# jackra1n/raytracer-rust

Hardware: NVIDIA B200
Metric: Mpaths/s (semesterbild 800x600x256spp, depth 30) (higher is better)
Workload: dtype f32

## Files before the change

### raytracer-rust_b200/csrc/pt_bvh8.h

```cpp
#pragma once
#include "pt_math.h"
#include "pt_types.h"

namespace pt {

struct MeshHit {
  float t;
  uint32_t tri;
  uint32_t order;
};

PT_HD float box_rcp(float x) {
#if defined(__CUDA_ARCH__)
  float r;
  asm("rcp.approx.ftz.f32 %0, %1;" : "=f"(r) : "f"(x));
  return r;
#else
  return 1.0f / x;
#endif
}

template <int J>
PT_HD float byte_as_unit_float(uint32_t packed) {
#if defined(__CUDA_ARCH__)
// ... 22 lines not shown
  uint32_t octinv;
  uint2 ng;
  uint2 tg;
  uint2 tg2;
};

PT_HD void trav_begin(TravState &s, V3 o, V3 d, float t_min, float t_max) {
  s.o = o;
  s.d = d;
  s.idx = box_rcp(d.x), s.idy = box_rcp(d.y), s.idz = box_rcp(d.z);
  s.t_min = t_min;
  s.best_t = t_max;
  s.best_order = 0u;
  s.best_tri = 0xffffffffu;
  const uint32_t sx = f2u(d.x) >> 31, sy = f2u(d.y) >> 31, sz = f2u(d.z) >> 31;
  s.octinv = 7u - (sx | (sy << 1) | (sz << 2));
  s.ng = make_uint2(0u, 0x80000000u);
  s.tg = make_uint2(0u, 0u);
  s.tg2 = make_uint2(0u, 0u);
}
PT_HD bool trav_has_node(const TravState &s) { return s.ng.y > 0x00FFFFFFu; }
PT_HD bool trav_has_tri(const TravState &s) { return s.tg.y != 0u; }

template <bool COUNT>
PT_HD void trav_node(const DMesh &m, TravState &s, uint2 *stack, int &sp, TraversalCounters *ctr) {
  const uint32_t hits = s.ng.y, imask = hits & 0xffu;
  const int bit = 31 - clz32(hits);
  s.ng.y &= ~(1u << bit);
  if (s.ng.y > 0x00FFFFFFu) stack[sp++] = s.ng;
  const uint32_t slot = (uint32_t)(bit - 24) ^ s.octinv;
  const uint32_t rel = (uint32_t)popc32(imask & ~(0xFFFFFFFFu << slot));
  const float4 *np = m.nodes + (size_t)(s.ng.x + rel) * 5;
  const float4 q0 = ldg4(np), q1 = ldg4(np + 1), q2 = ldg4(np + 2), q3 = ldg4(np + 3), q4 = ldg4(np + 4);
  if (COUNT) ctr->nodes++;

  const uint32_t e = f2u(q0.w);
  const float adjx = u2f(((e & 0xffu) + 15u) << 23) * s.idx;
  const float adjy = u2f((((e >> 8) & 0xffu) + 15u) << 23) * s.idy;
  const float adjz = u2f((((e >> 16) & 0xffu) + 15u) << 23) * s.idz;
  const float orgx = (q0.x - s.o.x) * s.idx - adjx, orgy = (q0.y - s.o.y) * s.idy - adjy, orgz = (q0.z - s.o.z) * s.idz - adjz;

  const bool sx = (f2u(s.d.x) >> 31) != 0u, sy = (f2u(s.d.y) >> 31) != 0u, sz = (f2u(s.d.z) >> 31) != 0u;
  const uint32_t lox0 = f2u(q2.x), lox1 = f2u(q2.y), loy0 = f2u(q2.z), loy1 = f2u(q2.w);
  const uint32_t loz0 = f2u(q3.x), loz1 = f2u(q3.y), hix0 = f2u(q3.z), hix1 = f2u(q3.w);
  const uint32_t hiy0 = f2u(q4.x), hiy1 = f2u(q4.y), hiz0 = f2u(q4.z), hiz1 = f2u(q4.w);
  const uint32_t nx[2] = {sx ? hix0 : lox0, sx ? hix1 : lox1}, fx[2] = {sx ? lox0 : hix0, sx ? lox1 : hix1};
  const uint32_t ny[2] = {sy ? hiy0 : loy0, sy ? hiy1 : loy1}, fy[2] = {sy ? loy0 : hiy0, sy ? loy1 : hiy1};
  const uint32_t nz[2] = {sz ? hiz0 : loz0, sz ? hiz1 : loz1}, fz[2] = {sz ? loz0 : hiz0, sz ? loz1 : hiz1};
  const uint32_t meta[2] = {f2u(q1.z), f2u(q1.w)};
  const uint32_t octinv4 = s.octinv * 0x01010101u;

  uint32_t hitmask = 0u;
#pragma unroll
  for (int h = 0; h < 2; h++) {
    const uint32_t meta4 = meta[h];
    const uint32_t is_inner4 = (meta4 & (meta4 << 1)) & 0x10101010u;
    const uint32_t inner_mask4 = (is_inner4 >> 4) * 0xffu;
    const uint32_t bit_index4 = (meta4 ^ (octinv4 & inner_mask4)) & 0x1f1f1f1fu;
    const uint32_t child_bits4 = (meta4 >> 5) & 0x07070707u;
#define PT_CHILD2(J)                                                                                                  \
  {                                                                                                                   \
    float tnx0, tnx1, tny0, tny1, tnz0, tnz1, tfx0, tfx1, tfy0, tfy1, tfz0, tfz1;                                     \
    fma2_bcast(tnx0, tnx1, byte_as_unit_float<J>(nx[h]), byte_as_unit_float<J + 1>(nx[h]), adjx, orgx);               \
    fma2_bcast(tny0, tny1, byte_as_unit_float<J>(ny[h]), byte_as_unit_float<J + 1>(ny[h]), adjy, orgy);               \
    fma2_bcast(tnz0, tnz1, byte_as_unit_float<J>(nz[h]), byte_as_unit_float<J + 1>(nz[h]), adjz, orgz);               \
    fma2_bcast(tfx0, tfx1, byte_as_unit_float<J>(fx[h]), byte_as_unit_float<J + 1>(fx[h]), adjx, orgx);               \
    fma2_bcast(tfy0, tfy1, byte_as_unit_float<J>(fy[h]), byte_as_unit_float<J + 1>(fy[h]), adjy, orgy);               \
    fma2_bcast(tfz0, tfz1, byte_as_unit_float<J>(fz[h]), byte_as_unit_float<J + 1>(fz[h]), adjz, orgz);               \
             \
    const float tn0 = fmaxf(fmaxf(tnx0, tny0), fmaxf(tnz0, s.t_min)), tf0 = fminf(fminf(tfx0, tfy0), fminf(tfz0, s.best_t)); \
    const float tn1 = fmaxf(fmaxf(tnx1, tny1), fmaxf(tnz1, s.t_min)), tf1 = fminf(fminf(tfx1, tfy1), fminf(tfz1, s.best_t)); \
    if (tn0 <= tf0) hitmask |= ((child_bits4 >> (8 * (J))) & 0xffu) << ((bit_index4 >> (8 * (J))) & 0xffu);           \
    if (tn1 <= tf1) hitmask |= ((child_bits4 >> (8 * (J + 1))) & 0xffu) << ((bit_index4 >> (8 * (J + 1))) & 0xffu);   \
  }
    PT_CHILD2(0) PT_CHILD2(2)
#undef PT_CHILD
  }
  s.ng.x = f2u(q1.x);
  s.ng.y = (hitmask & 0xFF000000u) | (e >> 24);
  const uint2 leaf_hits = make_uint2(f2u(q1.y), hitmask & 0x00FFFFFFu);
  if (s.tg.y == 0u) s.tg = leaf_hits;
  else s.tg2 = leaf_hits;
}

template <bool COUNT>
PT_HD void trav_tri(const DMesh &m, TravState &s, TraversalCounters *ctr) {
  const int bit = 31 - clz32(s.tg.y);
  const float4 *tp = m.tris + (size_t)(s.tg.x + (uint32_t)bit) * 3;
  s.tg.y &= ~(1u << bit);
  if (s.tg.y == 0u) {
    s.tg = s.tg2;
    s.tg2 = make_uint2(0u, 0u);
  }
  const float4 t0 = ldg4(tp), t1 = ldg4(tp + 1), t2 = ldg4(tp + 2);
  if (COUNT) ctr->tris++;
  const V3 v0 = v3(t0.x, t0.y, t0.z), edge1 = v3(t1.x, t1.y, t1.z), edge2 = v3(t2.x, t2.y, t2.z);
  const V3 h = cross(s.d, edge2);
  const float a = dot(edge1, h);
  if (fabsf(a) < kEps) return;
  const float f = 1.0f / a;
  const V3 sv = s.o - v0;
  const float u = f * dot(sv, h);
  if (!(0.0f <= u && u <= 1.0f)) return;
  const V3 q = cross(sv, edge1);
  const float v = f * dot(s.d, q);
  if (v < 0.0f || u + v > 1.0f) return;
  const float t = f * dot(edge2, q);
  if (!(t > s.t_min)) return;
  const uint32_t order = f2u(t1.w);
  if (t < s.best_t || (t == s.best_t && order < s.best_order)) {
    s.best_t = t;
    s.best_order = order;
    s.best_tri = f2u(t0.w);
  }
}

template <bool COUNT>
PT_HD bool bvh8_closest(const DMesh &m, V3 o, V3 d, float t_min, float t_max, MeshHit &out, TraversalCounters *ctr) {
  TravState s;
  trav_begin(s, o, d, t_min, t_max);
  uint2 stack[kTraversalStack];
  int sp = 0;
  for (;;) {
    if (trav_has_tri(s)) {
      trav_tri<COUNT>(m, s, ctr);
    } else if (trav_has_node(s)) {
      trav_node<COUNT>(m, s, stack, sp, ctr);
    } else {
      if (sp == 0) break;
      s.ng = stack[--sp];
    }
  }
  if (s.best_tri == 0xffffffffu) return false;
  out.t = s.best_t;
  out.tri = s.best_tri;
  out.order = s.best_order;
  return true;
}

}
```

### raytracer-rust_b200/csrc/pt_prims.h

```cpp
#pragma once
#include "pt_bvh8.h"
#include "pt_math.h"
#include "pt_types.h"

namespace pt {

PT_HD void set_face_normal(Hit &h, V3 ray_d, V3 outward) {
  bool front = dot(ray_d, outward) < 0.0f;
  V3 n = front ? outward : -outward;
  h.front_face = front ? 1 : 0;
  h.nx = n.x;
  h.ny = n.y;
  h.nz = n.z;
}
PT_HD void set_pos(Hit &h, V3 p) {
  h.px = p.x;
  h.py = p.y;
  h.pz = p.z;
}

PT_HD bool hit_sphere(const float *f, const Ray &ray, float t_min, float t_max, Hit &h) {
  const float4 cr = ld4(reinterpret_cast<const float4 *>(f));
  const V3 center = v3(cr.x, cr.y, cr.z);
  const float radius = cr.w;
// ... 102 lines not shown
    }
  }
  const M4 w2o = load_m4(f);
  const V3 nw = normalized(mat_t_vector(w2o, n));
  set_face_normal(h, ray.d, nw);
}
PT_HD bool hit_cube(const float *f, const Ray &ray, float t_min, float t_max, Hit &h) {
  if (!hit_cube_t(f, ray, t_min, t_max, h)) return false;
  cube_finish_normal(f, ray, h);
  return true;
}

struct MeshRay {
  V3 o, d_raw, d;
};
template <bool PACKED = true>
PT_HD MeshRay mesh_object_ray(const float *w2o_f, const Ray &ray) {
  const M4 w2o = load_m4(w2o_f);
  MeshRay r;
  mat_point_vector<PACKED>(w2o, ray.o, ray.d, r.o, r.d_raw);
  r.d = normalized(normalized(r.d_raw));
  return r;
}
PT_HD bool mesh_root_may_hit(const DMesh &mesh, const MeshRay &r, float t_min, float t_max) {
  const float idx = box_rcp(r.d.x), idy = box_rcp(r.d.y), idz = box_rcp(r.d.z);
  const float ax = (mesh.root_lo[0] - r.o.x) * idx, bx = (mesh.root_hi[0] - r.o.x) * idx;
  const float ay = (mesh.root_lo[1] - r.o.y) * idy, by = (mesh.root_hi[1] - r.o.y) * idy;
  const float az = (mesh.root_lo[2] - r.o.z) * idz, bz = (mesh.root_hi[2] - r.o.z) * idz;
  const float tn = fmaxf(fmaxf(fminf(ax, bx), fminf(ay, by)), fmaxf(fminf(az, bz), t_min));
  const float tf = fminf(fminf(fmaxf(ax, bx), fmaxf(ay, by)), fminf(fmaxf(az, bz), t_max));
  return tn <= tf;
}

PT_HD bool mesh_finish(const float *f, float4 nq, const Ray &ray, const MeshRay &mr, const MeshHit &mh, float t_min, float t_max,
                       Hit &h) {
  const M4 w2o = load_m4(f), o2w = load_m4(f + 16);
  const V3 o = mr.o, d = mr.d;
  const V3 p_obj = o + d * mh.t;
  V3 n_obj = v3(nq.x, nq.y, nq.z);
  if (!(dot(d, n_obj) < 0.0f)) n_obj = -n_obj;
  const V3 pw = mat_point(o2w, p_obj);
  const V3 nw = normalized(mat_t_vector(w2o, n_obj));
  const float t_world = mh.t * length(mr.d_raw) / length(ray.d);
  if (t_world < t_min || t_world > t_max) return false;
  h.t = t_world;
  h.triangle = (int32_t)mh.tri;
  set_pos(h, pw);
  set_face_normal(h, ray.d, nw);
  return true;
}

PT_HD bool mesh_finish(const float *f, const DMesh &mesh, const Ray &ray, const MeshRay &mr, const MeshHit &mh, float t_min,
                       float t_max, Hit &h) {
  return mesh_finish(f, ldg4(mesh.normals + mh.order), ray, mr, mh, t_min, t_max, h);
// ... 44 lines not shown
```

### raytracer-rust_b200/csrc/pt_wavefront.cuh

```cuda
#pragma once
#include <cuda_runtime.h>

#include "../../include/ptcore.h"
#include "pt_adaptive.h"
#include "pt_bsdf.h"
#include "pt_philox.h"
#include "pt_prims.h"

namespace ptw {
using namespace pt;

constexpr int kBlock = 256;
constexpr int kSegPerSM = 4;
constexpr uint32_t kRefillLanes = 8;
constexpr uint32_t kNoSteal = 0x80000000u;
constexpr unsigned long long kNoTriHit = ~0ull;

struct Ctl {
  unsigned long long next_path;
  unsigned long long total_paths;
  unsigned long long rays;
  unsigned long long nodes, tris, mesh_rays;
  uint32_t n_active;
  uint32_t sync_timeouts;
  uint32_t iterations[2];
};

struct SegRange {
  uint32_t seg0;
  uint32_t n_seg;
  uint32_t half;
  uint32_t trav_seq, trav_parts;
  uint32_t *flags;
  uint32_t stage_id;
  uint32_t flag_wait;
  uint32_t *trav_counter;
};

struct RenderParams {
  DCamera cam;
  int32_t width, height;
  int32_t max_depth;
  int32_t sample_begin, n_samples;
  int32_t tiles_x, n_my_tiles, tile_mod, tile_rem;
  uint32_t row_mult;
  uint64_t seed;
  const uint32_t *pixel_list;
  uint32_t n_list;
};

struct Buffers {
  float4 *ray_o;
  float4 *ray_d;
  float4 *beta;
// ... 70 lines not shown
    const int type = ob->type;
    bool hit;
    if (type == OBJ_MESH) {
      const MeshRay mr = mesh_object_ray(ob->f, ray);
      if (!mesh_root_may_hit(sc.meshes[ob->mesh], mr, t_min, closest)) continue;
      park_ray = mr;
      return k;
    }
    if (type == OBJ_SPHERE) hit = hit_sphere(ob->f, ray, t_min, closest, best);
    else if (type == OBJ_QUAD) hit = hit_quad(ob->f, ray, t_min, closest, best);
    else if (type == OBJ_CUBE) hit = hit_cube_t(ob->f, ray, t_min, closest, best);
    else hit = hit_plane(ob->f, ray, t_min, closest, best);
    if (hit) {
      improved = true;
      closest = best.t;
      best.object = k;
      best.triangle = -1;
      best.material = ob->hit_bits;
    }
  }
  return -1;
}

__device__ __forceinline__ void finish_hit(const DObject *objs, const Ray &ray, Hit &best) {
  if (best.front_face == kCubeNormalPending) cube_finish_normal(objs[best.object].f, ray, best);
}

constexpr int kSmemObjects = 24;
template <bool kSharedObjs>
__device__ __forceinline__ const DObject *stage_objects(const DScene &sc, DObject *s_objs) {
  if (!kSharedObjs) return sc.objects;
  const uint4 *src = reinterpret_cast<const uint4 *>(sc.objects);
  uint4 *dst = reinterpret_cast<uint4 *>(s_objs);
  const int n16 = sc.n_objects * (int)(sizeof(DObject) / 16);
  for (int i = threadIdx.x; i < n16; i += blockDim.x) dst[i] = src[i];
  return s_objs;
}

__device__ __forceinline__ void park_tasks(uint32_t *s_ntask, const TaskQ &tq, int par, uint32_t seg_base, int park, uint32_t i,
                                           const MeshRay &mr, float closest) {
  const uint32_t lane = threadIdx.x & 31u;
  const uint32_t mask = __ballot_sync(0xffffffffu, park >= 0);
  if (mask == 0u) return;
  uint32_t slot0 = 0;
  if (lane == 0) slot0 = atomicAdd(s_ntask, (uint32_t)__popc(mask));
  slot0 = __shfl_sync(0xffffffffu, slot0, 0);
  if (park >= 0) {
    const uint32_t slot = seg_base + slot0 + (uint32_t)__popc(mask & ((1u << lane) - 1u));
    tq.ray[par][slot] = make_uint2(i, (uint32_t)park);
    tq.o[par][slot] = make_float4(mr.o.x, mr.o.y, mr.o.z, closest);
    tq.d[par][slot] = make_float4(mr.d.x, mr.d.y, mr.d.z, 0.0f);
    tq.res[par][slot] = kNoTriHit;
  }
}

template <bool kSharedObjs>
__device__ __forceinline__ void stage_pre(uint32_t seg, uint32_t n_seg, const DScene &sc, const ExtendOut &out, const TaskQ &tq,
                                          float t_min, float t_max) {
  __shared__ uint32_t s_ntask;
  __shared__ __align__(16) DObject s_objs[kSmemObjects];
  const uint32_t tid = threadIdx.x;
  const uint32_t n = out.b.cnt[seg], seg_base = seg * out.b.cap;
  if (tid == 0) s_ntask = 0;
  const DObject *objs = kSharedObjs ? s_objs : sc.objects;
  stage_objects<kSharedObjs>(sc, s_objs);
  __syncthreads();
  for (uint32_t c0 = 0; c0 < n; c0 += (uint32_t)kBlock) {
    const uint32_t i = seg_base + c0 + tid;
    int park = -1;
    MeshRay mr;
    float closest = t_max;
    if (c0 + tid < n) {
      const float4 o4 = out.b.ray_o[i], d4 = out.b.ray_d[i];
      const Ray ray{v3(o4.x, o4.y, o4.z), v3(d4.x, d4.y, d4.z)};
      Hit best;
      bool improved = false;
      park = scan_objects(sc, objs, ray, t_min, closest, best, improved, 0, mr);
      if (improved) finish_hit(objs, ray, best);
      if (improved) write_hit(out, i, best);
      else write_miss(out, i);
    }
    park_tasks(&s_ntask, tq, 0, seg_base, park, i, mr, closest);
  }
  __syncthreads();
  if (tid == 0 && tq.cnt) tq.cnt[seg] = s_ntask;
  (void)n_seg;
}

template <bool COUNT>
__device__ __forceinline__ void stage_traverse(uint32_t seg, uint32_t n_seg, Ctl *ctl, const DScene &sc, const TaskQ &tq, int round,
                                               float t_min, uint32_t cap, uint32_t refill_arg, uint32_t part = 0u, uint32_t parts = 1u) {
  __shared__ uint32_t s_cur;
  const uint32_t n_all = tq.cnt[(uint32_t)round * n_seg + seg];
  const uint32_t first = (uint32_t)((unsigned long long)n_all * part / parts);
  const uint32_t n = (uint32_t)((unsigned long long)n_all * (part + 1u) / parts) - first, seg_base = seg * cap + first;
  const int par = round & 1;
  const uint32_t lane = threadIdx.x & 31u;
  const uint32_t lt_mask = (1u << lane) - 1u;
  const uint32_t refill_lanes = refill_arg & ~kNoSteal;
  const bool steal = (refill_arg & kNoSteal) == 0u;
  const uint32_t quota = (n >= (uint32_t)kBlock || !steal) ? 32u : max(1u, (n + (uint32_t)(kBlock / 32) - 1u) / (uint32_t)(kBlock / 32));
  if (threadIdx.x == 0) s_cur = 0;
  __syncthreads();
  TraversalCounters tc{0u, 0u, 0u};
  TravState s;
  DMesh mesh;
  mesh.nodes = nullptr, mesh.tris = nullptr;
  uint2 stack[kTraversalStack];
  int sp = 0, sb = 0;
  bool active = false;
  uint32_t task = 0;
  bool exhausted = n == 0u;
  s.ng = make_uint2(0u, 0u);
  for (;;) {
    const uint32_t idle = __ballot_sync(0xffffffffu, !active);
    if (!exhausted && (idle == 0xffffffffu || (uint32_t)__popc(idle) >= refill_lanes)) {
      const uint32_t cnt = min((uint32_t)__popc(idle), quota);
      uint32_t base = 0;
      if (lane == 0) base = atomicAdd(&s_cur, cnt);
      base = __shfl_sync(0xffffffffu, base, 0);
      const uint32_t my_rank = (uint32_t)__popc(idle & lt_mask);
      if (!active && my_rank < cnt) {
        const uint32_t j = base + my_rank;
        if (j < n) {
          const uint32_t slot = seg_base + j;
          const uint2 rk = tq.ray[par][slot];
          const float4 o4 = tq.o[par][slot], d4 = __ldcs(&tq.d[par][slot]);
          const DMesh *gm = sc.meshes + sc.objects[rk.y].mesh;
          mesh.nodes = gm->nodes;
          mesh.tris = gm->tris;
          trav_begin(s, v3(o4.x, o4.y, o4.z), v3(d4.x, d4.y, d4.z), t_min, o4.w);
          sp = sb = 0;
          task = slot;
          active = true;
          if (COUNT) tc.mesh_rays++;
        }
      }
      if (base + cnt >= n) exhausted = true;
    } else if (steal && exhausted && idle != 0u && idle != 0xffffffffu) {
      const bool can_give = active && (sp > sb || __popc(s.ng.y >> 24) >= 2);
      const uint32_t donors = __ballot_sync(0xffffffffu, can_give);
      if (donors != 0u) {
        const uint32_t pairs = (uint32_t)min(__popc(idle), __popc(donors));
        const bool give = can_give && (uint32_t)__popc(donors & lt_mask) < pairs;
        const uint32_t my_idle_rank = (uint32_t)__popc(idle & lt_mask);
        const bool take = !active && my_idle_rank < pairs;
        uint2 entry = make_uint2(0u, 0u);
        if (give) {
          if (sp > sb) {
            entry = stack[sb++];
          } else {
            const uint32_t pend = s.ng.y & 0xFF000000u, bit = pend & (0u - pend);
            entry = make_uint2(s.ng.x, bit | (s.ng.y & 0xffu));
            s.ng.y &= ~bit;
          }
        }
        const int src = take ? (int)__fns(donors, 0u, (int)my_idle_rank + 1) : (int)lane;
        const float ox = __shfl_sync(0xffffffffu, s.o.x, src), oy = __shfl_sync(0xffffffffu, s.o.y, src), oz = __shfl_sync(0xffffffffu, s.o.z, src);
// ... 15 lines not shown
          mesh.nodes = reinterpret_cast<const float4 *>(pn);
          mesh.tris = reinterpret_cast<const float4 *>(ptri);
          task = tk;
          sp = sb = 0;
          active = true;
        }
      }
    }
    if (__ballot_sync(0xffffffffu, active) == 0u) {
      if (exhausted) break;
      continue;
    }
    if (active) {
      if (!trav_has_node(s)) {
        if (sp > sb) {
          s.ng = stack[--sp];
        } else if (!trav_has_tri(s)) {
          if (s.best_tri != 0xffffffffu) atomicMin(&tq.res[par][task], ((unsigned long long)f2u(s.best_t) << 32) | (unsigned long long)s.best_order);
          active = false;
          s.ng.y = 0u;
        }
        if (sp == sb) sp = sb = 0;
      }
      if (active && trav_has_node(s) && s.tg2.y == 0u) trav_node<COUNT>(mesh, s, stack, sp, &tc);
      if (active && trav_has_tri(s)) trav_tri<COUNT>(mesh, s, &tc);
    }
  }
  if (COUNT) {
    atomicAdd(&ctl->nodes, (unsigned long long)tc.nodes);
    atomicAdd(&ctl->tris, (unsigned long long)tc.tris);
    atomicAdd(&ctl->mesh_rays, (unsigned long long)tc.mesh_rays);
  }
}

template <bool kSharedObjs>
__device__ __forceinline__ void stage_post(uint32_t seg, uint32_t n_seg, const DScene &sc, const ExtendOut &out, const TaskQ &tq,
                                           int round, float t_min, float t_max) {
  __shared__ uint32_t s_ntask;
  __shared__ __align__(16) DObject s_objs[kSmemObjects];
  const uint32_t tid = threadIdx.x;
  const uint32_t n = tq.cnt[(uint32_t)round * n_seg + seg], seg_base = seg * out.b.cap;
  const int par = round & 1;
  if (tid == 0) s_ntask = 0;
  const DObject *objs = kSharedObjs ? s_objs : sc.objects;
  stage_objects<kSharedObjs>(sc, s_objs);
  __syncthreads();
  for (uint32_t c0 = 0; c0 < n; c0 += (uint32_t)kBlock) {
    const uint32_t j = seg_base + c0 + tid;
    int park = -1;
    MeshRay mr;
    float closest = t_max;
    uint32_t i = 0;
    if (c0 + tid < n) {
      const uint2 rk = tq.ray[par][j];
      const unsigned long long res = tq.res[par][j];
      i = rk.x;
      const int k = (int)rk.y;
      const DObject *ob = objs + k;
      const bool tri_hit = res != kNoTriHit;
      const uint32_t order = (uint32_t)res;
      const float4 o4 = out.b.ray_o[i], d4 = out.b.ray_d[i];
      closest = tq.o[par][j].w;
      float4 nq = make_float4(0.0f, 0.0f, 0.0f, 0.0f);
      if (tri_hit) nq = ldg4(sc.meshes[ob->mesh].normals + order);
      const Ray ray{v3(o4.x, o4.y, o4.z), v3(d4.x, d4.y, d4.z)};
      Hit best;
      best.triangle = -1;
      bool improved = false;
      if (tri_hit) {
        const MeshRay omr = mesh_object_ray<false>(ob->f, ray);
        MeshHit mh;
        mh.t = u2f((uint32_t)(res >> 32)), mh.tri = f2u(nq.w), mh.order = order;
        Hit tmp;
        if (mesh_finish(ob->f, nq, ray, omr, mh, t_min, closest, tmp)) {
          improved = true;
          closest = tmp.t;
          best = tmp;
          best.object = k;
          best.material = ob->hit_bits;
        }
      }
      park = scan_objects(sc, objs, ray, t_min, closest, best, improved, k + 1, mr);
      if (improved) finish_hit(objs, ray, best);
      if (improved) write_hit(out, i, best);
    }
    park_tasks(&s_ntask, tq, par ^ 1, seg_base, park, i, mr, closest);
  }
  __syncthreads();
  if (tid == 0) tq.cnt[(uint32_t)(round + 1) * n_seg + seg] = s_ntask;
}

constexpr int kShadeClasses = 11;
constexpr int kShadeWindow = 2048;
constexpr int kShadeGroups = kShadeWindow / kBlock;

__device__ __forceinline__ uint32_t block_rank(bool flag, uint32_t *s_warp , uint32_t *total) {
  const uint32_t lane = threadIdx.x & 31u, warp = threadIdx.x >> 5;
  const uint32_t mask = __ballot_sync(0xffffffffu, flag);
  if (lane == 0) s_warp[warp] = (uint32_t)__popc(mask);
  __syncthreads();
  if (threadIdx.x == 0) {
    uint32_t tot = 0;
    for (int w = 0; w < kBlock / 32; w++) {
      const uint32_t c = s_warp[w];
      s_warp[w] = tot;
      tot += c;
    }
    s_warp[kBlock / 32] = tot;
  }
  __syncthreads();
  *total = s_warp[kBlock / 32];
  return s_warp[warp] + (uint32_t)__popc(mask & ((1u << lane) - 1u));
// ... 307 lines not shown
  else segment_wait(sr, seg, ctl);
}
__device__ __forceinline__ void stage_end(const SegRange &sr, uint32_t seg) {
  if (sr.flags == nullptr) return;
  __syncthreads();
  if (threadIdx.x == 0) st_release_u32(sr.flags + seg, sr.stage_id);
}

__global__ void __launch_bounds__(kBlock, kSegPerSM) k_extend_pre(Ctl *ctl, SegRange sr, DScene sc, ExtendOut out, TaskQ tq, float t_min,
                                                                  float t_max, volatile uint32_t *progress, uint32_t seq) {
  const uint32_t seg = sr.seg0 + blockIdx.x;
  stage_begin(sr, seg, ctl);
  if (threadIdx.x == 0) {
    const uint32_t n = out.b.cnt[seg];
    if (n) {
      atomicAdd(&ctl->rays, (unsigned long long)n);
      atomicMax(&ctl->iterations[0], seq);
    }
    if (progress && blockIdx.x == 0) {
      *progress = seq << 2 | (ctl->next_path >= ctl->total_paths ? 2u : 0u) | (ctl->n_active == 0u ? 1u : 0u);
      __threadfence_system();
    }
  }
  if (sc.n_objects <= kSmemObjects) stage_pre<true>(seg, sr.n_seg, sc, out, tq, t_min, t_max);
  else stage_pre<false>(seg, sr.n_seg, sc, out, tq, t_min, t_max);
  stage_end(sr, seg);
}
template <bool COUNT>
__global__ void __launch_bounds__(kBlock, kSegPerSM) k_traverse(Ctl *ctl, SegRange sr, DScene sc, TaskQ tq, int round, float t_min,
                                                                uint32_t cap, uint32_t refill_lanes) {
  if (sr.trav_parts <= 1u) {
    stage_begin(sr, sr.seg0 + blockIdx.x, ctl);
    stage_traverse<COUNT>(sr.seg0 + blockIdx.x, sr.n_seg, ctl, sc, tq, round, t_min, cap, refill_lanes);
    stage_end(sr, sr.seg0 + blockIdx.x);
    return;
  }
  asm volatile("griddepcontrol.launch_dependents;" ::: "memory");
  if (sr.flags == nullptr || sr.flag_wait == 0u) asm volatile("griddepcontrol.wait;" ::: "memory");
  __shared__ uint32_t s_item;
  if (threadIdx.x == 0) s_item = blockIdx.x;
  __syncthreads();
  for (;;) {
    {
      const uint32_t item = s_item;
      if (item >= sr.n_seg * sr.trav_parts) break;
      const uint32_t seg = sr.seg0 + item % sr.n_seg;
      segment_wait(sr, seg, ctl);
      stage_traverse<COUNT>(seg, sr.n_seg, ctl, sc, tq, round, t_min, cap, refill_lanes, item / sr.n_seg, sr.trav_parts);
    }
    __syncthreads();
    if (threadIdx.x == 0) {
      if (sr.flags) {
        const uint32_t seg = sr.seg0 + s_item % sr.n_seg;
        __threadfence();
        if (atomicInc(sr.flags + 2u * sr.n_seg + seg, sr.trav_parts - 1u) == sr.trav_parts - 1u) {
          __threadfence();
          st_release_u32(sr.flags + seg, sr.stage_id);
        }
      }
      s_item = gridDim.x + atomicAdd(sr.trav_counter, 1u);
    }
    __syncthreads();
  }
}
__global__ void __launch_bounds__(kBlock, kSegPerSM) k_extend_post(Ctl *ctl, SegRange sr, DScene sc, ExtendOut out, TaskQ tq, int round,
                                                                   float t_min, float t_max) {
  stage_begin(sr, sr.seg0 + blockIdx.x, ctl);
  if (sc.n_objects <= kSmemObjects) stage_post<true>(sr.seg0 + blockIdx.x, sr.n_seg, sc, out, tq, round, t_min, t_max);
  else stage_post<false>(sr.seg0 + blockIdx.x, sr.n_seg, sc, out, tq, round, t_min, t_max);
  stage_end(sr, sr.seg0 + blockIdx.x);
}
template <int Mode, bool List = false>
__global__ void __launch_bounds__(kBlock, kSegPerSM) k_shade(Ctl *ctl, SegRange sr, DScene sc, RenderParams rp, Buffers b, Film film) {
  stage_begin(sr, sr.seg0 + blockIdx.x, ctl);
  stage_shade<Mode, List>(sr.seg0 + blockIdx.x, sr.n_seg, sr.flags ? sr.flags + sr.n_seg : nullptr, ctl, sc, rp, b, film);
  stage_end(sr, sr.seg0 + blockIdx.x);
}

__global__ void k_film_to_accum(Film film, size_t n_pixels, float *accum) {
  const size_t i = (size_t)blockIdx.x * blockDim.x + threadIdx.x;
  if (i >= n_pixels * 3) return;
  const size_t px = i / 3;
  accum[i] += film_value(film.sum[i], film.flags[px], (int)(i - px * 3));
}
__global__ void k_resolve(const float *rgb, size_t n_pixels, float scale, uint32_t *out) {
  const size_t i = (size_t)blockIdx.x * blockDim.x + threadIdx.x;
  if (i < n_pixels) out[i] = resolve_pixel(rgb[i * 3] * scale, rgb[i * 3 + 1] * scale, rgb[i * 3 + 2] * scale);
}
__global__ void k_resolve_film(Film film, size_t n_pixels, float scale, const int32_t *counts, float *rgb, uint32_t *packed) {
  const size_t p = (size_t)blockIdx.x * blockDim.x + threadIdx.x;
  if (p >= n_pixels) return;
  if (counts) scale = 1.0f / (float)counts[p];
// ... 122 lines not shown
```

### raytracer-rust_b200/csrc/ptcore.cu

```cuda
#include <cuda_runtime.h>
#include <dlfcn.h>
#include <nccl.h>

#include <algorithm>
#include <chrono>
#include <memory>
#include <mutex>
#include <thread>
#include <cstdio>
#include <cstdlib>
#include <cstring>
#include <deque>
#include <functional>
#include <string>
#include <vector>

#include <cub/device/device_select.cuh>

#include "../../include/ptcore.h"
#include "pt_build_dev.h"
#include "pt_scene_host.h"
#include "pt_wavefront.cuh"

using namespace pt;
// ... 167 lines not shown
constexpr int kTravParts = 4;

enum Stage { ST_PRE = 0, ST_TRAVERSE, ST_POST, ST_SHADE, ST_COUNT };

template <typename... KArgs, typename... Args>
void launch_stage(bool pdl, cudaStream_t stream, uint32_t segments, void (*kernel)(KArgs...), Args &&...args) {
  cudaLaunchAttribute attr;
  attr.id = cudaLaunchAttributeProgrammaticStreamSerialization;
  attr.val.programmaticStreamSerializationAllowed = 1;
  cudaLaunchConfig_t cfg;
  memset(&cfg, 0, sizeof(cfg));
  cfg.gridDim = dim3(segments), cfg.blockDim = dim3(kBlock), cfg.dynamicSmemBytes = 0, cfg.stream = stream;
  cfg.attrs = pdl ? &attr : nullptr, cfg.numAttrs = pdl ? 1 : 0;
  CK(cudaLaunchKernelEx(&cfg, kernel, std::forward<Args>(args)...));
}

uint32_t traverse_refill_arg() {
  const char *r = getenv("PTC_REFILL"), *st = getenv("PTC_STEAL");
  return (r ? (uint32_t)atoi(r) : kRefillLanes) | ((st && atoi(st) == 0) ? kNoSteal : 0u);
}

int launch_extend(cudaStream_t stream, uint32_t segments, int rounds, Ctl *ctl, const DScene &ds, const ExtendOut &eo, const TaskQ &tq,
                  float t_min, float t_max, bool counters) {
  const SegRange sr{0u, segments, 0u, 0u, 1u};
  k_extend_pre<<<segments, kBlock, 0, stream>>>(ctl, sr, ds, eo, tq, t_min, t_max, nullptr, 0u);
  for (int r = 0; r < rounds; r++) {
    const SegRange tsr{0u, segments, 0u, (uint32_t)r, 1u};
    if (counters) k_traverse<true><<<segments, kBlock, 0, stream>>>(ctl, tsr, ds, tq, r, t_min, eo.b.cap, traverse_refill_arg());
    else k_traverse<false><<<segments, kBlock, 0, stream>>>(ctl, tsr, ds, tq, r, t_min, eo.b.cap, traverse_refill_arg());
    k_extend_post<<<segments, kBlock, 0, stream>>>(ctl, sr, ds, eo, tq, r, t_min, t_max);
  }
  return 1 + 2 * rounds;
}

void require_committed(const ptc_scene *s) {
  if (!s) throw std::invalid_argument("null scene");
  if (!s->committed) throw std::logic_error("scene not committed (call ptc_scene_commit first)");
}

void check_render_args(const ptc_camera *cam, const ptc_render_settings *st, bool has_output) {
  if (!cam || !st || !has_output) throw std::invalid_argument("null argument");
  if (st->width <= 0 || st->height <= 0 || st->spp <= 0) throw std::invalid_argument("bad render settings");
  if ((int64_t)st->width * st->height > (int64_t)0x3fffffff) throw std::invalid_argument("image too large");
  if ((st->flags & PTC_FLAG_NEE_SKY) && !(st->flags & PTC_FLAG_NEE)) throw std::invalid_argument("PTC_FLAG_NEE_SKY needs PTC_FLAG_NEE");
}

void sample_range(const ptc_render_settings *st, int &begin, int &end) {
// ... 128 lines not shown
    if (tev_used == s->timing_events.size()) {
      cudaEvent_t e;
      CK(cudaEventCreate(&e));
      s->timing_events.push_back(e);
    }
    return s->timing_events[tev_used++];
  };
  std::vector<int> mark_stage;
  const auto mark = [&](int stage) {
    CK(cudaEventRecord(tev(), stream));
    mark_stage.push_back(stage);
  };

  CK(cudaEventRecord(ev_begin, stream));
  uint64_t launches = 0;
  const uint32_t refill = traverse_refill_arg();
  auto is_done = [](const Ctl &c) { return c.n_active == 0 && c.sync_timeouts == 0 && c.next_path >= c.total_paths; };
  static const bool pdl_on = getenv("PTC_PDL") ? atoi(getenv("PTC_PDL")) != 0 : true;
  const bool pdl = pdl_on && !timing;
  if (init.total_paths != 0) {
    const bool dataflow = getenv("PTC_DATAFLOW") ? atoi(getenv("PTC_DATAFLOW")) != 0 : true;
    uint32_t stage_id = 0;
    auto seg_range = [&](uint32_t trav_seq_, uint32_t trav_parts_) {
      SegRange r{0u, segments, 0u, trav_seq_, trav_parts_, s->ws.seg_flags.p, ++stage_id, (dataflow && stage_id > 1u) ? 1u : 0u, nullptr};
      if (trav_parts_ > 1u) r.trav_counter = s->ws.trav_counters.p + trav_seq_;
      return r;
    };
    int64_t mesh_tris = 0;
    for (const auto &mb : s->hs.meshes) mesh_tris += mb->n;
    const char *tp_env = getenv("PTC_TRAV_PARTS");
    const uint32_t trav_parts_bulk = tp_env ? (uint32_t)std::max(1, atoi(tp_env)) : (mesh_tris >= kHeavyMeshTriangles ? (uint32_t)kTravParts : 1u);
    if (trav_parts_bulk > 1u) CK(cudaMemsetAsync(s->ws.trav_counters.p, 0, kTravCounters * sizeof(uint32_t), stream));
    uint32_t trav_seq = 0;
    bool draining = false;
    int flip = 0;
    const bool progress_on = getenv("PTC_PROGRESS") ? atoi(getenv("PTC_PROGRESS")) != 0 : true;
    uint32_t *d_progress = nullptr;
    if (progress_on) {
      CK(cudaHostGetDevicePointer((void **)&d_progress, s->h_progress, 0));
      *(volatile uint32_t *)s->h_progress = 0u;
    }
    uint64_t it = 0;
    auto run_extend = [&]() {
      const ExtendOut eo{bufs[flip], nullptr};
      if (timing) mark(ST_PRE);
      launch_stage(pdl, stream, segments, k_extend_pre, s->d_ctl.p, seg_range(0u, 1u), s->ds, eo, tq, kEps, INFINITY,
                   (volatile uint32_t *)d_progress, (uint32_t)(it + 1));
// ... 910 lines not shown
```

Measured before the change: 3168.

## Test mesh BVH root node during object scan before parking traversal tasks

The extend pre/post stages now run the full 8-wide root-node child test inline, from a shared-memory copy of each mesh's root node, before parking a ray as a traversal task. Rays that hit no root child skip the mesh entirely and continue scanning further objects. Parked tasks carry the precomputed root hit mask, so the traversal kernel enters the root directly instead of reloading and retesting it. This removes task-queue writes and traversal work for rays that miss every child, at the cost of extra ALU work and shared-memory staging in the extend stages, plus a looped object scan that may diverge within warps.

```diff
diff --git a/raytracer-rust_b200/csrc/pt_bvh8.h b/raytracer-rust_b200/csrc/pt_bvh8.h
--- a/raytracer-rust_b200/csrc/pt_bvh8.h
+++ b/raytracer-rust_b200/csrc/pt_bvh8.h
@@ -68,6 +68,69 @@
 PT_HD bool trav_has_node(const TravState &s) { return s.ng.y > 0x00FFFFFFu; }
 PT_HD bool trav_has_tri(const TravState &s) { return s.tg.y != 0u; }
 
+struct NodeWords {
+  float4 q0, q1, q2, q3, q4;
+  PT_HD uint32_t w(int i) const {
+    const float4 &q = i < 4 ? q0 : i < 8 ? q1 : i < 12 ? q2 : i < 16 ? q3 : q4;
+    const int c = i & 3;
+    return f2u(c == 0 ? q.x : c == 1 ? q.y : c == 2 ? q.z : q.w);
+  }
+};
+struct NodePtr {
+  const uint32_t *p;
+  PT_HD uint32_t w(int i) const { return p[i]; }
+};
+
+template <class Node>
+PT_HD uint32_t node_hits(const TravState &s, const Node &nd) {
+  const uint32_t e = nd.w(3);
+  const float adjx = u2f(((e & 0xffu) + 15u) << 23) * s.idx;
+  const float adjy = u2f((((e >> 8) & 0xffu) + 15u) << 23) * s.idy;
+  const float adjz = u2f((((e >> 16) & 0xffu) + 15u) << 23) * s.idz;
+  const float orgx = (u2f(nd.w(0)) - s.o.x) * s.idx - adjx, orgy = (u2f(nd.w(1)) - s.o.y) * s.idy - adjy,
+              orgz = (u2f(nd.w(2)) - s.o.z) * s.idz - adjz;
+
+  const bool sx = (f2u(s.d.x) >> 31) != 0u, sy = (f2u(s.d.y) >> 31) != 0u, sz = (f2u(s.d.z) >> 31) != 0u;
+  const uint32_t octinv4 = s.octinv * 0x01010101u;
+
+  uint32_t hitmask = 0u;
+#pragma unroll
+  for (int h = 0; h < 2; h++) {
+    const uint32_t lox = nd.w(8 + h), loy = nd.w(10 + h), loz = nd.w(12 + h), hix = nd.w(14 + h), hiy = nd.w(16 + h), hiz = nd.w(18 + h);
+    const uint32_t nx = sx ? hix : lox, fx = sx ? lox : hix, ny = sy ? hiy : loy, fy = sy ? loy : hiy, nz = sz ? hiz : loz, fz = sz ? loz : hiz;
+    const uint32_t meta4 = nd.w(6 + h);
+    const uint32_t is_inner4 = (meta4 & (meta4 << 1)) & 0x10101010u;
+    const uint32_t inner_mask4 = (is_inner4 >> 4) * 0xffu;
+    const uint32_t bit_index4 = (meta4 ^ (octinv4 & inner_mask4)) & 0x1f1f1f1fu;
+    const uint32_t child_bits4 = (meta4 >> 5) & 0x07070707u;
+#define PT_CHILD2(J)                                                                                                  \
+  {                                                                                                                   \
+    float tnx0, tnx1, tny0, tny1, tnz0, tnz1, tfx0, tfx1, tfy0, tfy1, tfz0, tfz1;                                     \
+    fma2_bcast(tnx0, tnx1, byte_as_unit_float<J>(nx), byte_as_unit_float<J + 1>(nx), adjx, orgx);                     \
+    fma2_bcast(tny0, tny1, byte_as_unit_float<J>(ny), byte_as_unit_float<J + 1>(ny), adjy, orgy);                     \
+    fma2_bcast(tnz0, tnz1, byte_as_unit_float<J>(nz), byte_as_unit_float<J + 1>(nz), adjz, orgz);                     \
+    fma2_bcast(tfx0, tfx1, byte_as_unit_float<J>(fx), byte_as_unit_float<J + 1>(fx), adjx, orgx);                     \
+    fma2_bcast(tfy0, tfy1, byte_as_unit_float<J>(fy), byte_as_unit_float<J + 1>(fy), adjy, orgy);                     \
+    fma2_bcast(tfz0, tfz1, byte_as_unit_float<J>(fz), byte_as_unit_float<J + 1>(fz), adjz, orgz);                     \
+             \
+    const float tn0 = fmaxf(fmaxf(tnx0, tny0), fmaxf(tnz0, s.t_min)), tf0 = fminf(fminf(tfx0, tfy0), fminf(tfz0, s.best_t)); \
+    const float tn1 = fmaxf(fmaxf(tnx1, tny1), fmaxf(tnz1, s.t_min)), tf1 = fminf(fminf(tfx1, tfy1), fminf(tfz1, s.best_t)); \
+    if (tn0 <= tf0) hitmask |= ((child_bits4 >> (8 * (J))) & 0xffu) << ((bit_index4 >> (8 * (J))) & 0xffu);           \
+    if (tn1 <= tf1) hitmask |= ((child_bits4 >> (8 * (J + 1))) & 0xffu) << ((bit_index4 >> (8 * (J + 1))) & 0xffu);   \
+  }
+    PT_CHILD2(0) PT_CHILD2(2)
+#undef PT_CHILD2
+  }
+  return hitmask;
+}
+
+PT_HD void trav_enter(TravState &s, uint32_t child_base, uint32_t tri_base, uint32_t imask, uint32_t hits) {
+  s.ng = make_uint2(child_base, (hits & 0xFF000000u) | imask);
+  const uint2 leaf_hits = make_uint2(tri_base, hits & 0x00FFFFFFu);
+  if (s.tg.y == 0u) s.tg = leaf_hits;
+  else s.tg2 = leaf_hits;
+}
+
 template <bool COUNT>
 PT_HD void trav_node(const DMesh &m, TravState &s, uint2 *stack, int &sp, TraversalCounters *ctr) {
   const uint32_t hits = s.ng.y, imask = hits & 0xffu;
@@ -77,56 +140,9 @@
   const uint32_t slot = (uint32_t)(bit - 24) ^ s.octinv;
   const uint32_t rel = (uint32_t)popc32(imask & ~(0xFFFFFFFFu << slot));
   const float4 *np = m.nodes + (size_t)(s.ng.x + rel) * 5;
-  const float4 q0 = ldg4(np), q1 = ldg4(np + 1), q2 = ldg4(np + 2), q3 = ldg4(np + 3), q4 = ldg4(np + 4);
+  const NodeWords nd{ldg4(np), ldg4(np + 1), ldg4(np + 2), ldg4(np + 3), ldg4(np + 4)};
   if (COUNT) ctr->nodes++;
-
-  const uint32_t e = f2u(q0.w);
-  const float adjx = u2f(((e & 0xffu) + 15u) << 23) * s.idx;
-  const float adjy = u2f((((e >> 8) & 0xffu) + 15u) << 23) * s.idy;
-  const float adjz = u2f((((e >> 16) & 0xffu) + 15u) << 23) * s.idz;
-  const float orgx = (q0.x - s.o.x) * s.idx - adjx, orgy = (q0.y - s.o.y) * s.idy - adjy, orgz = (q0.z - s.o.z) * s.idz - adjz;
-
-  const bool sx = (f2u(s.d.x) >> 31) != 0u, sy = (f2u(s.d.y) >> 31) != 0u, sz = (f2u(s.d.z) >> 31) != 0u;
-  const uint32_t lox0 = f2u(q2.x), lox1 = f2u(q2.y), loy0 = f2u(q2.z), loy1 = f2u(q2.w);
-  const uint32_t loz0 = f2u(q3.x), loz1 = f2u(q3.y), hix0 = f2u(q3.z), hix1 = f2u(q3.w);
-  const uint32_t hiy0 = f2u(q4.x), hiy1 = f2u(q4.y), hiz0 = f2u(q4.z), hiz1 = f2u(q4.w);
-  const uint32_t nx[2] = {sx ? hix0 : lox0, sx ? hix1 : lox1}, fx[2] = {sx ? lox0 : hix0, sx ? lox1 : hix1};
-  const uint32_t ny[2] = {sy ? hiy0 : loy0, sy ? hiy1 : loy1}, fy[2] = {sy ? loy0 : hiy0, sy ? loy1 : hiy1};
-  const uint32_t nz[2] = {sz ? hiz0 : loz0, sz ? hiz1 : loz1}, fz[2] = {sz ? loz0 : hiz0, sz ? loz1 : hiz1};
-  const uint32_t meta[2] = {f2u(q1.z), f2u(q1.w)};
-  const uint32_t octinv4 = s.octinv * 0x01010101u;
-
-  uint32_t hitmask = 0u;
-#pragma unroll
-  for (int h = 0; h < 2; h++) {
-    const uint32_t meta4 = meta[h];
-    const uint32_t is_inner4 = (meta4 & (meta4 << 1)) & 0x10101010u;
-    const uint32_t inner_mask4 = (is_inner4 >> 4) * 0xffu;
-    const uint32_t bit_index4 = (meta4 ^ (octinv4 & inner_mask4)) & 0x1f1f1f1fu;
-    const uint32_t child_bits4 = (meta4 >> 5) & 0x07070707u;
-#define PT_CHILD2(J)                                                                                                  \
-  {                                                                                                                   \
-    float tnx0, tnx1, tny0, tny1, tnz0, tnz1, tfx0, tfx1, tfy0, tfy1, tfz0, tfz1;                                     \
-    fma2_bcast(tnx0, tnx1, byte_as_unit_float<J>(nx[h]), byte_as_unit_float<J + 1>(nx[h]), adjx, orgx);               \
-    fma2_bcast(tny0, tny1, byte_as_unit_float<J>(ny[h]), byte_as_unit_float<J + 1>(ny[h]), adjy, orgy);               \
-    fma2_bcast(tnz0, tnz1, byte_as_unit_float<J>(nz[h]), byte_as_unit_float<J + 1>(nz[h]), adjz, orgz);               \
-    fma2_bcast(tfx0, tfx1, byte_as_unit_float<J>(fx[h]), byte_as_unit_float<J + 1>(fx[h]), adjx, orgx);               \
-    fma2_bcast(tfy0, tfy1, byte_as_unit_float<J>(fy[h]), byte_as_unit_float<J + 1>(fy[h]), adjy, orgy);               \
-    fma2_bcast(tfz0, tfz1, byte_as_unit_float<J>(fz[h]), byte_as_unit_float<J + 1>(fz[h]), adjz, orgz);               \
-             \
-    const float tn0 = fmaxf(fmaxf(tnx0, tny0), fmaxf(tnz0, s.t_min)), tf0 = fminf(fminf(tfx0, tfy0), fminf(tfz0, s.best_t)); \
-    const float tn1 = fmaxf(fmaxf(tnx1, tny1), fmaxf(tnz1, s.t_min)), tf1 = fminf(fminf(tfx1, tfy1), fminf(tfz1, s.best_t)); \
-    if (tn0 <= tf0) hitmask |= ((child_bits4 >> (8 * (J))) & 0xffu) << ((bit_index4 >> (8 * (J))) & 0xffu);           \
-    if (tn1 <= tf1) hitmask |= ((child_bits4 >> (8 * (J + 1))) & 0xffu) << ((bit_index4 >> (8 * (J + 1))) & 0xffu);   \
-  }
-    PT_CHILD2(0) PT_CHILD2(2)
-#undef PT_CHILD
-  }
-  s.ng.x = f2u(q1.x);
-  s.ng.y = (hitmask & 0xFF000000u) | (e >> 24);
-  const uint2 leaf_hits = make_uint2(f2u(q1.y), hitmask & 0x00FFFFFFu);
-  if (s.tg.y == 0u) s.tg = leaf_hits;
-  else s.tg2 = leaf_hits;
+  trav_enter(s, f2u(nd.q1.x), f2u(nd.q1.y), f2u(nd.q0.w) >> 24, node_hits(s, nd));
 }
 
 template <bool COUNT>
@@ -168,14 +184,12 @@
   uint2 stack[kTraversalStack];
   int sp = 0;
   for (;;) {
-    if (trav_has_tri(s)) {
-      trav_tri<COUNT>(m, s, ctr);
-    } else if (trav_has_node(s)) {
-      trav_node<COUNT>(m, s, stack, sp, ctr);
-    } else {
-      if (sp == 0) break;
-      s.ng = stack[--sp];
+    if (!trav_has_node(s)) {
+      if (sp > 0) s.ng = stack[--sp];
+      else if (!trav_has_tri(s)) break;
     }
+    if (trav_has_node(s) && s.tg2.y == 0u) trav_node<COUNT>(m, s, stack, sp, ctr);
+    if (trav_has_tri(s)) trav_tri<COUNT>(m, s, ctr);
   }
   if (s.best_tri == 0xffffffffu) return false;
   out.t = s.best_t;
diff --git a/raytracer-rust_b200/csrc/pt_prims.h b/raytracer-rust_b200/csrc/pt_prims.h
--- a/raytracer-rust_b200/csrc/pt_prims.h
+++ b/raytracer-rust_b200/csrc/pt_prims.h
@@ -148,14 +148,18 @@
   r.d = normalized(normalized(r.d_raw));
   return r;
 }
+PT_HD bool mesh_root_may_hit(const DMesh &mesh, const TravState &s) {
+  const float ax = (mesh.root_lo[0] - s.o.x) * s.idx, bx = (mesh.root_hi[0] - s.o.x) * s.idx;
+  const float ay = (mesh.root_lo[1] - s.o.y) * s.idy, by = (mesh.root_hi[1] - s.o.y) * s.idy;
+  const float az = (mesh.root_lo[2] - s.o.z) * s.idz, bz = (mesh.root_hi[2] - s.o.z) * s.idz;
+  const float tn = fmaxf(fmaxf(fminf(ax, bx), fminf(ay, by)), fmaxf(fminf(az, bz), s.t_min));
+  const float tf = fminf(fminf(fmaxf(ax, bx), fmaxf(ay, by)), fminf(fmaxf(az, bz), s.best_t));
+  return tn <= tf;
+}
 PT_HD bool mesh_root_may_hit(const DMesh &mesh, const MeshRay &r, float t_min, float t_max) {
-  const float idx = box_rcp(r.d.x), idy = box_rcp(r.d.y), idz = box_rcp(r.d.z);
-  const float ax = (mesh.root_lo[0] - r.o.x) * idx, bx = (mesh.root_hi[0] - r.o.x) * idx;
-  const float ay = (mesh.root_lo[1] - r.o.y) * idy, by = (mesh.root_hi[1] - r.o.y) * idy;
-  const float az = (mesh.root_lo[2] - r.o.z) * idz, bz = (mesh.root_hi[2] - r.o.z) * idz;
-  const float tn = fmaxf(fmaxf(fminf(ax, bx), fminf(ay, by)), fmaxf(fminf(az, bz), t_min));
-  const float tf = fminf(fminf(fmaxf(ax, bx), fmaxf(ay, by)), fminf(fmaxf(az, bz), t_max));
-  return tn <= tf;
+  TravState s;
+  trav_begin(s, r.o, r.d, t_min, t_max);
+  return mesh_root_may_hit(mesh, s);
 }
 
 PT_HD bool mesh_finish(const float *f, float4 nq, const Ray &ray, const MeshRay &mr, const MeshHit &mh, float t_min, float t_max,
diff --git a/raytracer-rust_b200/csrc/pt_wavefront.cuh b/raytracer-rust_b200/csrc/pt_wavefront.cuh
--- a/raytracer-rust_b200/csrc/pt_wavefront.cuh
+++ b/raytracer-rust_b200/csrc/pt_wavefront.cuh
@@ -29,7 +29,7 @@
 struct SegRange {
   uint32_t seg0;
   uint32_t n_seg;
-  uint32_t half;
+  uint32_t count;
   uint32_t trav_seq, trav_parts;
   uint32_t *flags;
   uint32_t stage_id;
@@ -146,23 +146,41 @@
   return -1;
 }
 
+__device__ __forceinline__ uint32_t root_hits(const DScene &sc, const float4 *roots, int mesh, const MeshRay &mr, float t_min, float closest) {
+  TravState rs;
+  trav_begin(rs, mr.o, mr.d, t_min, closest);
+  const float4 *rn = roots ? roots + 5 * mesh : sc.meshes[mesh].nodes;
+  return node_hits(rs, NodePtr{reinterpret_cast<const uint32_t *>(rn)});
+}
+
 __device__ __forceinline__ void finish_hit(const DObject *objs, const Ray &ray, Hit &best) {
   if (best.front_face == kCubeNormalPending) cube_finish_normal(objs[best.object].f, ray, best);
 }
 
 constexpr int kSmemObjects = 24;
+__device__ __forceinline__ bool shared_objects(const DScene &sc) { return sc.n_objects <= kSmemObjects && sc.n_meshes <= kSmemObjects; }
 template <bool kSharedObjs>
-__device__ __forceinline__ const DObject *stage_objects(const DScene &sc, DObject *s_objs) {
-  if (!kSharedObjs) return sc.objects;
+__device__ __forceinline__ void stage_objects(const DScene &sc, DObject *s_objs, float4 *s_roots) {
+  if (!kSharedObjs) return;
   const uint4 *src = reinterpret_cast<const uint4 *>(sc.objects);
   uint4 *dst = reinterpret_cast<uint4 *>(s_objs);
   const int n16 = sc.n_objects * (int)(sizeof(DObject) / 16);
   for (int i = threadIdx.x; i < n16; i += blockDim.x) dst[i] = src[i];
-  return s_objs;
+  for (int i = threadIdx.x; i < sc.n_meshes * 5; i += blockDim.x) s_roots[i] = sc.meshes[i / 5].nodes[i % 5];
+}
+
+__device__ __forceinline__ void count_roots(uint32_t *s_sum, uint32_t n_roots) {
+  const uint32_t w = __reduce_add_sync(0xffffffffu, n_roots);
+  if ((threadIdx.x & 31u) == 0u && w != 0u) atomicAdd(s_sum, w);
+}
+__device__ __forceinline__ void flush_roots(Ctl *ctl, uint32_t n) {
+  if (n == 0u) return;
+  atomicAdd(&ctl->nodes, (unsigned long long)n);
+  atomicAdd(&ctl->mesh_rays, (unsigned long long)n);
 }
 
 __device__ __forceinline__ void park_tasks(uint32_t *s_ntask, const TaskQ &tq, int par, uint32_t seg_base, int park, uint32_t i,
-                                           const MeshRay &mr, float closest) {
+                                           const MeshRay &mr, uint32_t hits, float closest) {
   const uint32_t lane = threadIdx.x & 31u;
   const uint32_t mask = __ballot_sync(0xffffffffu, park >= 0);
   if (mask == 0u) return;
@@ -173,41 +191,53 @@
     const uint32_t slot = seg_base + slot0 + (uint32_t)__popc(mask & ((1u << lane) - 1u));
     tq.ray[par][slot] = make_uint2(i, (uint32_t)park);
     tq.o[par][slot] = make_float4(mr.o.x, mr.o.y, mr.o.z, closest);
-    tq.d[par][slot] = make_float4(mr.d.x, mr.d.y, mr.d.z, 0.0f);
+    tq.d[par][slot] = make_float4(mr.d.x, mr.d.y, mr.d.z, u2f(hits));
     tq.res[par][slot] = kNoTriHit;
   }
 }
 
 template <bool kSharedObjs>
-__device__ __forceinline__ void stage_pre(uint32_t seg, uint32_t n_seg, const DScene &sc, const ExtendOut &out, const TaskQ &tq,
-                                          float t_min, float t_max) {
-  __shared__ uint32_t s_ntask;
+__device__ __forceinline__ void stage_pre(uint32_t seg, uint32_t n_seg, Ctl *ctl, bool count, const DScene &sc, const ExtendOut &out,
+                                          const TaskQ &tq, float t_min, float t_max) {
+  __shared__ uint32_t s_ntask, s_roots_tested;
   __shared__ __align__(16) DObject s_objs[kSmemObjects];
+  __shared__ float4 s_roots[kSmemObjects * 5];
   const uint32_t tid = threadIdx.x;
   const uint32_t n = out.b.cnt[seg], seg_base = seg * out.b.cap;
-  if (tid == 0) s_ntask = 0;
+  if (tid == 0) s_ntask = 0, s_roots_tested = 0;
   const DObject *objs = kSharedObjs ? s_objs : sc.objects;
-  stage_objects<kSharedObjs>(sc, s_objs);
+  stage_objects<kSharedObjs>(sc, s_objs, s_roots);
   __syncthreads();
   for (uint32_t c0 = 0; c0 < n; c0 += (uint32_t)kBlock) {
     const uint32_t i = seg_base + c0 + tid;
     int park = -1;
     MeshRay mr;
+    uint32_t hits = 0u, n_roots = 0u;
     float closest = t_max;
     if (c0 + tid < n) {
       const float4 o4 = out.b.ray_o[i], d4 = out.b.ray_d[i];
       const Ray ray{v3(o4.x, o4.y, o4.z), v3(d4.x, d4.y, d4.z)};
-      Hit best;
-      bool improved = false;
-      park = scan_objects(sc, objs, ray, t_min, closest, best, improved, 0, mr);
-      if (improved) finish_hit(objs, ray, best);
-      if (improved) write_hit(out, i, best);
-      else write_miss(out, i);
-    }
-    park_tasks(&s_ntask, tq, 0, seg_base, park, i, mr, closest);
+      for (int k = 0;;) {
+        Hit best;
+        bool improved = false;
+        park = scan_objects(sc, objs, ray, t_min, closest, best, improved, k, mr);
+        if (improved) finish_hit(objs, ray, best);
+        if (improved) write_hit(out, i, best);
+        else if (k == 0) write_miss(out, i);
+        if (park < 0) break;
+        n_roots++;
+        hits = root_hits(sc, kSharedObjs ? s_roots : nullptr, objs[park].mesh, mr, t_min, closest);
+        if (hits != 0u) break;
+        k = park + 1;
+        park = -1;
+      }
+    }
+    if (count) count_roots(&s_roots_tested, n_roots);
+    park_tasks(&s_ntask, tq, 0, seg_base, park, i, mr, hits, closest);
   }
   __syncthreads();
   if (tid == 0 && tq.cnt) tq.cnt[seg] = s_ntask;
+  if (tid == 0 && count) flush_roots(ctl, s_roots_tested);
   (void)n_seg;
 }
 
@@ -233,6 +263,7 @@
   uint2 stack[kTraversalStack];
   int sp = 0, sb = 0;
   bool active = false;
+  bool entered = false;
   uint32_t task = 0;
   bool exhausted = n == 0u;
   s.ng = make_uint2(0u, 0u);
@@ -254,10 +285,12 @@
           mesh.nodes = gm->nodes;
           mesh.tris = gm->tris;
           trav_begin(s, v3(o4.x, o4.y, o4.z), v3(d4.x, d4.y, d4.z), t_min, o4.w);
+          const float4 r0 = ldg4(mesh.nodes), r1 = ldg4(mesh.nodes + 1);
+          trav_enter(s, f2u(r1.x), f2u(r1.y), f2u(r0.w) >> 24, f2u(d4.w));
+          entered = true;
           sp = sb = 0;
           task = slot;
           active = true;
-          if (COUNT) tc.mesh_rays++;
         }
       }
       if (base + cnt >= n) exhausted = true;
@@ -319,33 +352,35 @@
         }
         if (sp == sb) sp = sb = 0;
       }
-      if (active && trav_has_node(s) && s.tg2.y == 0u) trav_node<COUNT>(mesh, s, stack, sp, &tc);
+      if (active && !entered && trav_has_node(s) && s.tg2.y == 0u) trav_node<COUNT>(mesh, s, stack, sp, &tc);
       if (active && trav_has_tri(s)) trav_tri<COUNT>(mesh, s, &tc);
+      entered = false;
     }
   }
   if (COUNT) {
     atomicAdd(&ctl->nodes, (unsigned long long)tc.nodes);
     atomicAdd(&ctl->tris, (unsigned long long)tc.tris);
-    atomicAdd(&ctl->mesh_rays, (unsigned long long)tc.mesh_rays);
   }
 }
 
 template <bool kSharedObjs>
-__device__ __forceinline__ void stage_post(uint32_t seg, uint32_t n_seg, const DScene &sc, const ExtendOut &out, const TaskQ &tq,
-                                           int round, float t_min, float t_max) {
-  __shared__ uint32_t s_ntask;
+__device__ __forceinline__ void stage_post(uint32_t seg, uint32_t n_seg, Ctl *ctl, bool count, const DScene &sc, const ExtendOut &out,
+                                           const TaskQ &tq, int round, float t_min, float t_max) {
+  __shared__ uint32_t s_ntask, s_roots_tested;
   __shared__ __align__(16) DObject s_objs[kSmemObjects];
+  __shared__ float4 s_roots[kSmemObjects * 5];
   const uint32_t tid = threadIdx.x;
   const uint32_t n = tq.cnt[(uint32_t)round * n_seg + seg], seg_base = seg * out.b.cap;
   const int par = round & 1;
-  if (tid == 0) s_ntask = 0;
+  if (tid == 0) s_ntask = 0, s_roots_tested = 0;
   const DObject *objs = kSharedObjs ? s_objs : sc.objects;
-  stage_objects<kSharedObjs>(sc, s_objs);
+  stage_objects<kSharedObjs>(sc, s_objs, s_roots);
   __syncthreads();
   for (uint32_t c0 = 0; c0 < n; c0 += (uint32_t)kBlock) {
     const uint32_t j = seg_base + c0 + tid;
     int park = -1;
     MeshRay mr;
+    uint32_t hits = 0u, n_roots = 0u;
     float closest = t_max;
     uint32_t i = 0;
     if (c0 + tid < n) {
@@ -377,14 +412,25 @@
           best.material = ob->hit_bits;
         }
       }
-      park = scan_objects(sc, objs, ray, t_min, closest, best, improved, k + 1, mr);
-      if (improved) finish_hit(objs, ray, best);
-      if (improved) write_hit(out, i, best);
-    }
-    park_tasks(&s_ntask, tq, par ^ 1, seg_base, park, i, mr, closest);
+      for (int kb = k + 1;;) {
+        park = scan_objects(sc, objs, ray, t_min, closest, best, improved, kb, mr);
+        if (improved) finish_hit(objs, ray, best);
+        if (improved) write_hit(out, i, best);
+        if (park < 0) break;
+        n_roots++;
+        hits = root_hits(sc, kSharedObjs ? s_roots : nullptr, objs[park].mesh, mr, t_min, closest);
+        if (hits != 0u) break;
+        kb = park + 1;
+        park = -1;
+        improved = false;
+      }
+    }
+    if (count) count_roots(&s_roots_tested, n_roots);
+    park_tasks(&s_ntask, tq, par ^ 1, seg_base, park, i, mr, hits, closest);
   }
   __syncthreads();
   if (tid == 0) tq.cnt[(uint32_t)(round + 1) * n_seg + seg] = s_ntask;
+  if (tid == 0 && count) flush_roots(ctl, s_roots_tested);
 }
 
 constexpr int kShadeClasses = 11;
@@ -738,8 +784,8 @@
       __threadfence_system();
     }
   }
-  if (sc.n_objects <= kSmemObjects) stage_pre<true>(seg, sr.n_seg, sc, out, tq, t_min, t_max);
-  else stage_pre<false>(seg, sr.n_seg, sc, out, tq, t_min, t_max);
+  if (shared_objects(sc)) stage_pre<true>(seg, sr.n_seg, ctl, sr.count != 0u, sc, out, tq, t_min, t_max);
+  else stage_pre<false>(seg, sr.n_seg, ctl, sr.count != 0u, sc, out, tq, t_min, t_max);
   stage_end(sr, seg);
 }
 template <bool COUNT>
@@ -782,8 +828,8 @@
 __global__ void __launch_bounds__(kBlock, kSegPerSM) k_extend_post(Ctl *ctl, SegRange sr, DScene sc, ExtendOut out, TaskQ tq, int round,
                                                                    float t_min, float t_max) {
   stage_begin(sr, sr.seg0 + blockIdx.x, ctl);
-  if (sc.n_objects <= kSmemObjects) stage_post<true>(sr.seg0 + blockIdx.x, sr.n_seg, sc, out, tq, round, t_min, t_max);
-  else stage_post<false>(sr.seg0 + blockIdx.x, sr.n_seg, sc, out, tq, round, t_min, t_max);
+  if (shared_objects(sc)) stage_post<true>(sr.seg0 + blockIdx.x, sr.n_seg, ctl, sr.count != 0u, sc, out, tq, round, t_min, t_max);
+  else stage_post<false>(sr.seg0 + blockIdx.x, sr.n_seg, ctl, sr.count != 0u, sc, out, tq, round, t_min, t_max);
   stage_end(sr, sr.seg0 + blockIdx.x);
 }
 template <int Mode, bool List = false>
diff --git a/raytracer-rust_b200/csrc/ptcore.cu b/raytracer-rust_b200/csrc/ptcore.cu
--- a/raytracer-rust_b200/csrc/ptcore.cu
+++ b/raytracer-rust_b200/csrc/ptcore.cu
@@ -213,7 +213,7 @@
 
 int launch_extend(cudaStream_t stream, uint32_t segments, int rounds, Ctl *ctl, const DScene &ds, const ExtendOut &eo, const TaskQ &tq,
                   float t_min, float t_max, bool counters) {
-  const SegRange sr{0u, segments, 0u, 0u, 1u};
+  const SegRange sr{0u, segments, counters ? 1u : 0u, 0u, 1u};
   k_extend_pre<<<segments, kBlock, 0, stream>>>(ctl, sr, ds, eo, tq, t_min, t_max, nullptr, 0u);
   for (int r = 0; r < rounds; r++) {
     const SegRange tsr{0u, segments, 0u, (uint32_t)r, 1u};
@@ -388,7 +388,7 @@
     const bool dataflow = getenv("PTC_DATAFLOW") ? atoi(getenv("PTC_DATAFLOW")) != 0 : true;
     uint32_t stage_id = 0;
     auto seg_range = [&](uint32_t trav_seq_, uint32_t trav_parts_) {
-      SegRange r{0u, segments, 0u, trav_seq_, trav_parts_, s->ws.seg_flags.p, ++stage_id, (dataflow && stage_id > 1u) ? 1u : 0u, nullptr};
+      SegRange r{0u, segments, counters ? 1u : 0u, trav_seq_, trav_parts_, s->ws.seg_flags.p, ++stage_id, (dataflow && stage_id > 1u) ? 1u : 0u, nullptr};
       if (trav_parts_ > 1u) r.trav_counter = s->ws.trav_counters.p + trav_seq_;
       return r;
     };
```

Measured after the change: 2923 (median of 6 runs). -7.7%, worse.
